# emmanuel-ferdman/pinot

Measured on AMD Instinct MI355X. Metric: rows scanned/s (G) + p50 query latency, SSB flattened SF100/SF1000, 1-8 GPU, higher is better.
Workload: dtype u32 dict ids / int64 sums; 1 GPU; SSB SF100 flattened lineorder per GPU, 100 segments x 6000000 rows, queries Q1.1+Q1.2+Q1.3; layout=sorted by LO_ORDERDATE (SURVEY.md §8d C2), rows_per_gpu=600000000, parallelism=one GPU (no collective)

## Files before the change

### pinot_amd/csrc/agg_kernel.h

```cpp
#pragma once
#include <hip/hip_ext.h>

#include "agg_common.h"

namespace phip {

struct HistCtx {
  lds_u32 *bins;
  int n;
};
template <int NA>
__device__ __forceinline__ void hist_flush(cquery_t &q, cseg_t &seg, uint64_t (&acc)[NA], HistCtx &hc) {
  const int lane = lane_id();
  ccol_t &c = seg.cols[q.hist_col];
#pragma unroll
  for (int a = 0; a < NA; a++) {
    if (a >= q.num_aggs) break;
    if (!((q.hist_aggs >> a) & 1u)) continue;
    const int kind = q.aggs[a].acc;
    if (kind == ACC_SUM_I64) {
      for (int i = lane; i < c.card; i += 64) {
        const uint32_t cnt = (hc.bins[i >> 1] >> ((i & 1) * 16)) & 0xffffu;
        if (cnt) acc[a] += (uint64_t)cnt * (uint64_t)dict_i64(c, (uint32_t)i);
      }
// ... 655 lines not shown
  }
  HistCtx hc{nullptr, 0};
  if constexpr (kHist) {
    hc.bins = (lds_u32 *)rest + (size_t)hll_words + (size_t)wave * q.hist_words;
    for (int i = lane; i < q.hist_words; i += 64) hc.bins[i] = 0;
  }
  if (MODE == GB_LDS) {
    const int G = (int)q.num_groups;
    for (int i = threadIdx.x; i < q.tbl_words; i += kBlock) {
      const int row = i / G;
      uint64_t init = 0;
      if (row > 0 && q.aggs[row - 1].acc == ACC_MIN_F64) init = ~0ull;
      tbl[i] = init;
    }
    for (int i = threadIdx.x; i < q.hll_words; i += kBlock) hll_packed[i] = 0;
  }
  __syncthreads();

  const int x = blockIdx.x & 7;
  const int j = blockIdx.x >> 3;
  const int gx = gridDim.x >> 3;
  const int xs = (int)((int64_t)q.total_work * x / 8);
  const int xe = (int)((int64_t)q.total_work * (x + 1) / 8);
  const int wx = gx * W;
  const int wid = j * W + wave;

  uint64_t acc[NA];
#pragma unroll
  for (int a = 0; a < NA; a++) acc[a] = (a < q.num_aggs) ? acc_init(q.aggs[a].acc) : 0;

  cseg_t *segs = (cseg_t *)q.segs;
  const glb_u32 *mask = (const glb_u32 *)q.mask;
  int head = 0, tail = 0;
  int si = 0;
  int dict_si = -1;
  int t = xs + wid;
  constexpr int kMaskAhead = 4;
  uint32_t mq[kMaskAhead];
#pragma unroll
  for (int k = 0; k < kMaskAhead; k++)
    mq[k] = (mask != nullptr && t + k * wx < xe) ? __builtin_nontemporal_load(mask + (size_t)(t + k * wx) * 64 + lane) : 0u;
  for (; t < xe; t += wx) {
    const uint32_t m_raw = mq[0];
#pragma unroll
    for (int k = 0; k + 1 < kMaskAhead; k++) mq[k] = mq[k + 1];
    {
      const int tn = t + kMaskAhead * wx;
      mq[kMaskAhead - 1] = (mask != nullptr && tn < xe) ? __builtin_nontemporal_load(mask + (size_t)tn * 64 + lane) : 0u;
    }
    if (segs[si].work_begin + segs[si].num_work <= t) {
      if constexpr (MODE == GB_NONE) {
        if (head > tail) agg_ring_batch<NA, kHist>(q, segs[si], ring, tail, head - tail, acc, hll_lds, 0, &hc);
        if constexpr (kHist) hist_flush<NA>(q, segs[si], acc, hc);
      } else if constexpr (kGbBatch) {
        if (head > tail) group_ring_batch<MODE, kBatch, kRingGB, kRec>(q, segs[si], ring, tail, head - tail, tbl, hll_packed);
      } else if (head > tail) {
        const bool act = lane < head - tail;
        const int32_t doc = act ? (int32_t)ring[(tail + lane) & (R - 1)] : 0;
        do_chunk<NA, MODE, kRec>(q, segs[si], doc, act, acc, hll_lds, tbl, hll_packed);
      }
      head = tail = 0;
      while (si + 1 < q.num_segs && segs[si + 1].work_begin <= t) si++;
    }
    cseg_t &seg = segs[si];
    const int32_t doc0 = (seg.tile0 + (t - seg.work_begin)) * kTileDocs;
    const int32_t nvalid = min(kTileDocs, seg.num_docs - doc0);
    const uint32_t valid = valid_word(nvalid, lane);
    const uint32_t m = mask != nullptr ? (m_raw & valid) : valid;
    bool dense = ballot(m != valid) == 0;
    if constexpr (MODE == GB_NONE && kDense) {
      if (!dense) dense = wave_sum_u32((uint32_t)__popc(m)) >= (uint32_t)q.dense_min;
    }
    bool batched = false;
    if constexpr (MODE == GB_NONE && kDense) batched = dense;
    if constexpr (MODE == GB_NONE && kDense) {
    if (batched) {
      if (q.num_stage > 0) {
        if (dict_si != si) {
          for (int k = 0; k < q.num_stage; k++) {
            if (q.stage_dict_off[k] < 0) continue;
            ccol_t &c = seg.cols[q.stage_col[k]];
            if (!c.has_dict) continue;
            const int32_t nw = c.card * ((c.type == PHIP_TYPE_LONG || c.type == PHIP_TYPE_DOUBLE) ? 2 : 1);
            lds_u32 *dst = (lds_u32 *)(stg + q.stage_dict_off[k]);
            for (int i = lane; i < nw; i += 64) dst[i] = ((const glb_u32 *)c.dict)[i];
          }
          dict_si = si;
        }
        const int32_t tile = doc0 / kTileDocs;
        for (int k = 0; k < q.num_stage; k++) {
          ccol_t &c = seg.cols[q.stage_col[k]];
          if (!c.has_dict) continue;
          const int32_t nb = 256 * c.bits;
          const uint8_t *src = (const uint8_t *)c.words + (size_t)tile * nb + lane * 16;
          const uint32_t dst = stg_lds + (uint32_t)q.stage_off[k];
// ... 141 lines not shown
```

### pinot_amd/csrc/dev_common.h

```cpp
#pragma once
#include <hip/hip_runtime.h>

#include "../../include/pinot_hip.h"
#include "acc_ops.h"
#include "device.h"

namespace phip {

#define PHIP_CAS __attribute__((address_space(4)))
#define PHIP_GLB __attribute__((address_space(1)))
#define PHIP_LDS __attribute__((address_space(3)))
typedef const PHIP_CAS DevSeg cseg_t;
typedef const PHIP_CAS DevNode cnode_t;
typedef const PHIP_CAS DevCol ccol_t;

__device__ __forceinline__ int lane_id() { return threadIdx.x & 63; }

__device__ __forceinline__ uint64_t ballot(bool p) { return __ballot(p); }

__device__ __forceinline__ uint32_t mbcnt64(uint64_t m) {
  return __builtin_amdgcn_mbcnt_hi((uint32_t)(m >> 32), __builtin_amdgcn_mbcnt_lo((uint32_t)m, 0u));
}

__device__ __forceinline__ int uniform(int v) { return __builtin_amdgcn_readfirstlane(v); }

typedef uint32_t u32x2_a4 __attribute__((ext_vector_type(2), aligned(4)));
__device__ __forceinline__ uint32_t decode_bits(const uint32_t *words_generic, uint64_t off, uint32_t bits) {
  const PHIP_GLB u32x2_a4 *p = (const PHIP_GLB u32x2_a4 *)((const PHIP_GLB uint32_t *)words_generic + (off >> 5));
  const u32x2_a4 v = __builtin_nontemporal_load(p);
  const uint64_t win = ((uint64_t)v.x << 32) | (uint64_t)v.y;
  return (uint32_t)((win << (off & 31)) >> (64 - bits));
}

__device__ __forceinline__ uint32_t window_at(const PHIP_LDS uint32_t *w, int32_t p) {
  const int32_t q = (p - 1) >> 5;
  const uint32_t s = (uint32_t)(32 * (q + 1) - p);
  return __builtin_amdgcn_alignbit(w[q], w[q + 1], s);
}

#ifndef PHIP_DMA_POLICY
#define PHIP_DMA_POLICY "nt"
#endif
__device__ __forceinline__ void dma16(const uint8_t *gsrc, uint32_t lds_dst) {
  unsigned keep;
  asm volatile(
      "s_mov_b32 %0, m0\n\t"
      "s_mov_b32 m0, %2\n\t"
// ... 112 lines not shown
```

### pinot_amd/csrc/device.h

```cpp
#pragma once
#include <stdint.h>

#if defined(__HIPCC__)
#define PHIP_HD __host__ __device__
#else
#define PHIP_HD
#endif

namespace phip {

constexpr int kMaxQueryColumns = 16;
constexpr int kMaxAggs = 8;
constexpr int kRecKeys = 4;
constexpr int kRecFields = kRecKeys + 2 * kMaxAggs;
enum { REC_BITS = 0, REC_U16 = 1, REC_U32 = 2 };
struct RecSrc {
  const void *p;
  int32_t kind, bits, off, pad;
};
struct RecSrcs {
  RecSrc f[kRecFields];
};
constexpr int kMaxPrograms = 8;
constexpr int kDenseMin = 640;
// ... 207 lines not shown
  const int32_t *kf;
  uint64_t *segm;
  uint32_t *hll;
  uint64_t *out;
  uint32_t *counter;
  int32_t nba, na, nbf, nseg, hll_words, pad;
};

struct DevFilter {
  const DevSeg *segs;
  const DevNode *nodes;
  int32_t num_segs;
  int32_t total_work;
  int32_t stage_stride;
  int32_t nbuf;
  int32_t xcd_walk;
  int32_t min_dma;
  int32_t probe;
  int32_t contig_inline;
  uint32_t stats_programs;
  int32_t mask_nt;
  uint32_t *mask_out;
  uint64_t *partials;
  uint64_t *seg_matched;
  const struct DevAggQuery *agg;
  uint64_t *agg_partials;
  int32_t fring_bytes;
  int32_t pad_f;
  const DevFinal *fin;
  uint64_t *rec;
  const int32_t *rec_first;
  int32_t rec_stride;
  uint32_t rec_tag;
};

struct DevAgg {
  int32_t acc;
  int32_t expr;
  int32_t col_a;
  int32_t col_b;
  int32_t integral;
  int32_t hll_slot;
  int32_t log2m;
  int32_t program;
};

struct DevAggQuery {
  const DevSeg *segs;
  int32_t num_segs;
  int32_t total_work;
  const uint32_t *mask;
  int32_t num_aggs;
  int32_t num_hll;
  int32_t log2m;
  int32_t mode;
  DevAgg aggs[kMaxAggs];
  int32_t num_group_by;
  int32_t gb_cols[kMaxGroupBy];
  int32_t dense_batch;
  int64_t gb_stride[kMaxGroupBy];
  int64_t num_groups;
  int32_t tbl_words;
  int32_t hll_words;
  uint64_t *gb_table;
  uint32_t *gb_hll;
  uint64_t *partials;
  uint32_t *hll_regs;
  int32_t stage_bytes;
  int32_t num_stage;
  int32_t stage_col[kMaxAggStage];
  int32_t stage_off[kMaxAggStage];
  int32_t stage_dict_off[kMaxAggStage];
  int32_t stage_slot_a[kMaxAggs];
  int32_t stage_slot_b[kMaxAggs];
  uint64_t *gb_keys;
  uint32_t *hash_overflow;
  int32_t seg_keys;
  int32_t seg_key_mult;
  uint32_t *first_doc;
  int32_t dense_min;
  int32_t own_count_rows;
  const DevFinal *fin;
  int32_t wg_waves;
  int32_t rec_on;
  int64_t xcd_words;
  int64_t xcd_hll_words;
  int8_t rec_fa[kMaxAggs];
  int8_t rec_fb[kMaxAggs];
  uint32_t hist_aggs;
  int32_t hist_col;
  int32_t hist_words;
  int32_t hist_pad;
};

constexpr int kMaxSelect = 16;
enum SelKind : int32_t {
  SEL_I64 = 0,
  SEL_F64 = 1,
  SEL_ID = 2,
  SEL_STR = 3,
};
struct DevSelect {
  int32_t expr;
  int32_t col_a;
  int32_t col_b;
  int32_t kind;
};
struct DevSelQuery {
  const DevSeg *segs;
  int32_t num_segs;
  int32_t total_work;
  const uint32_t *mask;
  const int64_t *tile_off;
  const int64_t *seg_base;
  int64_t limit;
  int32_t num_select;
  int32_t pad;
  DevSelect sel[kMaxSelect];
};

constexpr int kMaxDistinct = kMaxAggs;
constexpr int kDistinctLdsWords = 8192;
constexpr int kCountsCombineCard = 64;
constexpr int kCountsCombineRounds = 16;
struct DevDistinctQuery {
  const DevSeg *segs;
  int32_t num_segs;
  int32_t total_work;
  const uint32_t *mask;
  uint32_t *bitmap;
  int64_t num_rows;
  int64_t row_words;
  int32_t num_slots;
  int32_t lds;
  int32_t slot_col[kMaxDistinct];
  int32_t slot_card[kMaxDistinct];
  int32_t slot_kind[kMaxDistinct];
  int64_t slot_off[kMaxDistinct];
  int32_t num_group_by;
  int32_t combine_card;
  int32_t combine_rounds;
  int32_t gb_cols[kMaxGroupBy];
  int64_t gb_stride[kMaxGroupBy];
};

constexpr int kMaxOrderKeys = 8;
struct KeyOrder {
  int32_t num_group_by;
  int32_t num_keys;
  int32_t gb[kMaxOrderKeys];
  int32_t desc[kMaxOrderKeys];
  int64_t card[kMaxOrderKeys];
};

enum OrderTermKind : int32_t { TERM_GROUP_KEY = 0, TERM_VALUE = 1, TERM_AVG = 2, TERM_RANGE = 3, TERM_HLL = 4 };
struct OrderTerms {
  int32_t num_group_by;
  int32_t num_terms;
  int64_t card[kMaxOrderKeys];
  int32_t kind[kMaxOrderKeys];
  int32_t a[kMaxOrderKeys];
  int32_t b[kMaxOrderKeys];
  int32_t desc[kMaxOrderKeys];
};

struct RawChunk {
  uint64_t src;
  uint64_t dst;
  uint32_t csize;
  uint32_t usize;
};

struct RoaringTask {
  const uint8_t *payload;
  uint64_t *out_words;
  int32_t key;
// ... 15 lines not shown
```

### pinot_amd/csrc/distinct.hip

```cpp
#include "agg_common.h"
#include "launch.h"

namespace phip {

typedef const PHIP_CAS DevDistinctQuery cdst_t;

constexpr int kDstBlock = 256;
constexpr int kDstWaves = kDstBlock / kWave;

__device__ __forceinline__ int32_t slot_words(cdst_t &q, int s) {
  return q.slot_kind[s] == PHIP_DISTINCT_SLOT_COUNTS ? q.slot_card[s] : (q.slot_card[s] + 31) >> 5;
}

__device__ __forceinline__ int64_t distinct_key(cdst_t &q, cseg_t &seg, int32_t doc) {
  int64_t key = 0;
  for (int k = 0; k < q.num_group_by; k++) {
    ccol_t &c = seg.cols[q.gb_cols[k]];
    const uint32_t id = col_dict_id(c, doc);
    const int64_t gid = c.remap ? ((const PHIP_GLB int32_t *)c.remap)[id] : (int32_t)id;
    key += gid * q.gb_stride[k];
  }
  return key;
}

__device__ __forceinline__ void mark_global(uint32_t *word, uint32_t bit) {
  glb_u32 *p = (glb_u32 *)word;
  if (__hip_atomic_load(p, PHIP_RLX, PHIP_AG) & bit) return;
  (void)__hip_atomic_fetch_or(p, bit, PHIP_RLX, PHIP_AG);
}

template <bool kLds>
__global__ __launch_bounds__(kDstBlock) void distinct_mark_kernel(const DevDistinctQuery *qp) {
  extern __shared__ uint32_t dst_lds[];
  cdst_t &q = *(cdst_t *)qp;
  cseg_t *segs = (cseg_t *)q.segs;
  const int lane = lane_id();
  const int wave = uniform(threadIdx.x >> 6);
  const int32_t row_words = (int32_t)q.row_words;
  if (kLds) {
    for (int32_t i = threadIdx.x; i < row_words; i += kDstBlock) dst_lds[i] = 0u;
    __syncthreads();
  }
  const int64_t nw = (int64_t)gridDim.x * kDstWaves, w = (int64_t)blockIdx.x * kDstWaves + wave;
  const int b = (int)((int64_t)q.total_work * w / nw), e = (int)((int64_t)q.total_work * (w + 1) / nw);
  int si = 0;
  for (int t = b; t < e; t++) {
    while (si + 1 < q.num_segs && segs[si + 1].work_begin <= t) si++;
    cseg_t &seg = segs[si];
    const int32_t doc0 = (seg.tile0 + (t - seg.work_begin)) * kTileDocs;
    const uint32_t valid = valid_word(min(kTileDocs, seg.num_docs - doc0), lane);
    const uint32_t m =
        q.mask != nullptr ? (((const PHIP_GLB uint32_t *)q.mask)[(size_t)t * 64 + lane] & valid) : valid;
    uint32_t any = wave_or32(m);
    while (any) {
      const int g = __builtin_clz(any);
      any &= ~(0x80000000u >> g);
      if (!((m << g) & 0x80000000u)) continue;
      const int32_t doc = doc0 + 64 * g + lane;
      const int64_t key = q.num_group_by > 0 ? distinct_key(q, seg, doc) : 0;
      if (key < 0 || key >= q.num_rows) continue;
      for (int s = 0; s < q.num_slots; s++) {
        ccol_t &c = seg.cols[q.slot_col[s]];
        const uint32_t id = col_dict_id(c, doc);
        const uint32_t gid = c.remap ? (uint32_t)((const PHIP_GLB int32_t *)c.remap)[id] : id;
        if (gid >= (uint32_t)q.slot_card[s]) continue;
        if (q.slot_kind[s] == PHIP_DISTINCT_SLOT_COUNTS) {
          const uint64_t w = (kLds ? 0ull : (uint64_t)key * (uint64_t)q.row_words) + (uint64_t)q.slot_off[s] + gid;
          uint32_t add = 1u;
          if (!kLds && q.slot_card[s] <= q.combine_card) {
            bool pending = true;
            for (int r = 0; r < q.combine_rounds && pending; r++) {
              const uint32_t lo = (uint32_t)__builtin_amdgcn_readfirstlane((int)(uint32_t)w);
              const uint32_t hi = (uint32_t)__builtin_amdgcn_readfirstlane((int)(uint32_t)(w >> 32));
              const bool mine = w == (((uint64_t)hi << 32) | lo);
              const uint64_t same = ballot(mine);
              if (mine) {
                add = mbcnt64(same) == 0 ? (uint32_t)__popcll(same) : 0u;
                pending = false;
              }
            }
// ... 77 lines not shown
```

### pinot_amd/csrc/filter_kernel.h

```cpp
#pragma once
#include <hip/hip_ext.h>

#include "agg_kernel.h"
#include "host_final.h"

namespace phip {

struct Tile {
  int32_t doc0;
  int32_t valid_docs;
  const PHIP_LDS uint8_t *stage;
};

#define PHIP_GROUP_LOOP(PASS_EXPR)                                             \
  const int lane = lane_id();                                                  \
  const int32_t p = lane * B;                                                  \
  const int32_t q = (p - 1) >> 5;                                              \
  const uint32_t s = (uint32_t)(32 * (q + 1) - p);                             \
  const PHIP_LDS uint32_t *wl = w + q;                                         \
  const int32_t gstride = 2 * B;                                               \
  uint32_t r = 0;                                                              \
  _Pragma("unroll 8") for (int g = 0; g < kTileGroups; g++) {                  \
    const uint32_t win = __builtin_amdgcn_alignbit(wl[0], wl[1], s);           \
    wl += gstride;                                                             \
// ... 1110 lines not shown
  const int head0 = head;
  const int npiece = head - tail + r.total <= kFusedRingGB ? 1 : 16;
  const int lanes = 64 / npiece;
  for (int p = 0; p < npiece; p++) {
    const int e = __builtin_amdgcn_readlane((int)r.incl, lanes * p + lanes - 1);
    write_ranked<uint32_t, kFusedRingGB>(r, lanes * p, lanes * (p + 1), -head0, t.doc0, ring);
    head = head0 + e;
    while (head - tail >= kGbFlush) {
      fused_flush_gb<MODE>(aq, seg, ring, tail, kGbFlush, tbl, hll_packed);
      tail += kGbFlush;
    }
  }
}

#define PHIP_VMW(k) \
  case k: asm volatile("s_waitcnt vmcnt(" #k ")" ::: "memory"); break;
__device__ __forceinline__ void wait_vmcnt_lb(int n) {
  switch (__builtin_amdgcn_readfirstlane(n)) {
    PHIP_VMW(0) PHIP_VMW(1) PHIP_VMW(2) PHIP_VMW(3) PHIP_VMW(4) PHIP_VMW(5) PHIP_VMW(6) PHIP_VMW(7)
    PHIP_VMW(8) PHIP_VMW(9) PHIP_VMW(10) PHIP_VMW(11) PHIP_VMW(12) PHIP_VMW(13) PHIP_VMW(14)
    default: asm volatile("s_waitcnt vmcnt(15)" ::: "memory"); break;
  }
}
#undef PHIP_VMW

template <int kS>
struct StageCursor {
  const uint8_t *ptr[kS];
  int32_t bytes[kS];
  int32_t lds[kS];
  int32_t n;
};

template <int kS>
__device__ __forceinline__ void cursor_load(StageCursor<kS> &c, cseg_t &seg, int32_t tile_in_seg) {
  c.n = seg.num_stage;
#pragma unroll
  for (int i = 0; i < kS; i++) {
    c.ptr[i] = nullptr;
    c.bytes[i] = 0;
    c.lds[i] = 0;
    if (i < c.n) {
      c.bytes[i] = seg.stage[i].bytes;
      c.lds[i] = seg.stage[i].lds_off;
      c.ptr[i] = seg.stage[i].base + (int64_t)tile_in_seg * c.bytes[i];
    }
  }
}

template <int kS>
__device__ __forceinline__ void cursor_issue(StageCursor<kS> &c, uint32_t lbase, int step) {
  const int lane16 = lane_id() * 16;
#pragma unroll
  for (int i = 0; i < kS; i++) {
    if (i < c.n) {
      const uint8_t *g = c.ptr[i] + lane16;
      const uint32_t l = lbase + (uint32_t)c.lds[i];
      const int32_t nb = c.bytes[i];
      for (int off = 0; off < nb; off += 1024) {
        if (off + lane16 < nb) dma16(g + off, l + (uint32_t)off);
      }
      c.ptr[i] += (int64_t)nb * step;
    }
  }
}

template <int NA>
__device__ __forceinline__ void record_store(const DevFilter &q, const uint64_t *part, const uint64_t *apart,
                                             const uint32_t *segrow) {
  const int i = (int)threadIdx.x;
  if (i >= (q.rec_stride >> 3)) return;
  int na = 0;
  if constexpr (NA > 0) na = ((cquery_t *)q.agg)->num_aggs;
  uint64_t v = 0;
  if (i < 2) {
    for (int w = 0; w < kFilterWaves; w++) v += part[w * 2 + i];
  } else if (i < 2 + 2 * na) {
    if constexpr (NA > 0) {
// ... 52 lines not shown
  const int st = kBsDefer ? 0 : (q.mask_out != nullptr ? 1 : 0);
  constexpr int NAX = NA > 0 ? NA : 1;
  constexpr int kB = kBsDefer ? lean_batch(NA) : kFusedBatch;
  constexpr int kGbMode = NA == kFusedGroupByXcd ? GB_XCD : (NA == kFusedGroupByLds ? GB_LDS : GB_GLOBAL);
  lds_u64 *gtbl = nullptr;
  lds_u32 *ghll = nullptr;
  if constexpr (NA == kFusedGroupByLds) {
    cquery_t &aq = *(cquery_t *)q.agg;
    gtbl = (lds_u64 *)(smem + (size_t)kFilterWaves * (nbuf * stride + q.fring_bytes));
    ghll = (lds_u32 *)((PHIP_LDS uint8_t *)gtbl + (size_t)aq.tbl_words * 8);
    const int G = (int)aq.num_groups;
    for (int i = threadIdx.x; i < aq.tbl_words; i += kFilterBlock) {
      const int row = i / G;
      gtbl[i] = (row > 0 && aq.aggs[row - 1].acc == ACC_MIN_F64) ? ~0ull : 0ull;
    }
    for (int i = threadIdx.x; i < aq.hll_words; i += kFilterBlock) ghll[i] = 0;
    __syncthreads();
  }
  __shared__ uint32_t segrow[kFilterWaves][NA >= 0 ? kRecSegSlots : 1];
  if constexpr (NA >= 0) {
    segrow[wave][min(lane, kRecSegSlots - 1)] = 0;
  }
  uint64_t acc[NAX];
  SmallDict sda[NAX], sdb[NAX];
  if constexpr (NA > 0) {
    cquery_t &aq = *(cquery_t *)q.agg;
#pragma unroll
    for (int a = 0; a < NA; a++) {
      acc[a] = a < aq.num_aggs ? acc_init(aq.aggs[a].acc) : 0;
      sda[a] = sdb[a] = SmallDict{0u, 0u, false};
    }
  }

  int pf = begin, pfc = 0, psn = 0, pend = -1, pslot = 0;
  StageCursor<kS> cur;
  cur.n = 0;
#define PHIP_PREFETCH()                                                                         \
  do {                                                                                          \
    if (pf >= pend) {                                                                           \
      while (psn + 1 < q.num_segs && segs[psn].work_begin + segs[psn].num_work <= pf) psn++;    \
      cseg_t &ps = segs[psn];                                                                   \
      pend = ps.work_begin + ps.num_work;                                                       \
      cursor_load<kS>(cur, ps, ps.tile0 + (pf - ps.work_begin));                                \
    }                                                                                           \
    cursor_issue<kS>(cur, ring_lds + (uint32_t)(pslot * stride), step);                         \
    pf += step;                                                                                 \
    pfc++;                                                                                      \
    pslot = pslot + 1 == nbuf ? 0 : pslot + 1;                                                  \
  } while (0)
  for (int i = 0; i < nbuf - 1 && pf < end; i++) PHIP_PREFETCH();

  int si = -1;
  int seg_end = -1;
  int slot = 0;
  int k = 0;
  for (int t = begin; t < end; t += step, k++) {
    if (pf < end) PHIP_PREFETCH();
    if (t >= seg_end) {
      if constexpr (NA > 0) {
        if (si >= 0 && dhead > dtail)
          fused_flush<NA, kB>(*(cquery_t *)q.agg, segs[si], deferring, dtail, dhead - dtail, sda, sdb, acc);
        dhead = dtail = 0;
      }
      if constexpr (NA < 0) {
        while (si >= 0 && dhead > dtail) {
          fused_flush_gb<kGbMode>(*(cquery_t *)q.agg, segs[si], deferring, dtail, min(dhead - dtail, kGbFlush), gtbl,
                                  ghll);
          dtail += kGbFlush;
        }
        dhead = dtail = 0;
      }
      if (si >= 0) {
        const uint64_t m = wave_reduce_u64_add(lane_matched);
        lane_matched = 0;
        matched_total += m;
        if (NA >= 0 && q.seg_matched == nullptr) {
          if (lane == 0) segrow[wave][si % kRecSegSlots] = (uint32_t)m;
        } else if (m && lane == 0) {
          atomicAdd((unsigned long long *)&q.seg_matched[segs[si].seg_index], (unsigned long long)m);
        }
      }
      si = si < 0 ? 0 : si;
      while (si + 1 < q.num_segs && segs[si + 1].work_begin <= t) si++;
      seg_end = segs[si].work_begin + segs[si].num_work;
      if constexpr (NA > 0) {
        cquery_t &aq = *(cquery_t *)q.agg;
#pragma unroll
        for (int a = 0; a < NA; a++) {
          if (a >= aq.num_aggs || aq.aggs[a].acc == ACC_COUNT) continue;
          sda[a] = load_small_dict(segs[si].cols[aq.aggs[a].col_a]);
          if (aq.aggs[a].expr != PHIP_EXPR_COLUMN) sdb[a] = load_small_dict(segs[si].cols[aq.aggs[a].col_b]);
        }
      }
    }
    cseg_t &seg = segs[si];
    Tile tl;
    const int32_t tile_in_seg = seg.tile0 + (t - seg.work_begin);
    tl.doc0 = tile_in_seg * kTileDocs;
    tl.valid_docs = min(kTileDocs, seg.num_docs - tl.doc0);
    tl.stage = ring + slot * stride;
    wait_vmcnt_lb((pfc - k - 1) * nd + min(k, nbuf - 1) * st);

    const uint32_t valid = valid_word(tl.valid_docs, lane);
    uint32_t scanned_t = 0;
    uint32_t mask;
    if (q.probe) {
      mask = valid;
    } else if (kConjOnly || seg.conj_path) {
      if constexpr (kBsDefer) mask = seg.conj > 0 ? (valid & eval_conj_bs(seg, tl.stage)) : valid;
      else mask = seg.conj > 0 ? eval_conj(seg, tl.stage, valid) : valid;
      if (seg.conj_range && (seg.conj_lo > tl.doc0 || seg.conj_hi < tl.doc0 + kTileDocs - 1)) {
        const int32_t lo = max(seg.conj_lo - tl.doc0, 0), hi = min(seg.conj_hi - tl.doc0, kTileDocs - 1);
        mask &= lo <= hi ? range_word(lo, hi, lane) : 0u;
      }
      scanned_t = (uint32_t)seg.conj * (uint32_t)tl.valid_docs;
// ... 118 lines not shown
```

### pinot_amd/csrc/runtime.cpp

```cpp
#include <hip/hip_runtime.h>

#include <algorithm>
#include <atomic>
#include <chrono>
#include <condition_variable>
#include <cmath>
#include <cstdarg>
#include <cstdio>
#include <cstring>
#include <functional>
#include <map>
#include <memory>
#include <mutex>
#include <string>
#include <unordered_map>
#include <vector>

#include "../../include/pinot_hip.h"
#include "device.h"
#include "host_final.h"
#include "launch.h"
#include "node.h"

using namespace phip;
// ... 3346 lines not shown
    num_entries++;
    if (hull_lo > hull_hi) continue;
    ds.tile0 = (int32_t)(hull_lo / kTileDocs);
    ds.num_work = (int32_t)(hull_hi / kTileDocs - ds.tile0 + 1);
    ds.work_begin = (int32_t)total_work;
    total_work += ds.num_work;
    dsegs.push_back(ds);
   }
  }
  if (hll_made) HIP_TRY(hipStreamSynchronize(st));
  if (total_work > INT32_MAX / 2) return fail(PHIP_ERR_UNSUPPORTED, "too many tiles in one query");
  dq.total_work = (int32_t)total_work;
  if (group_by && gb_key_space > ((int64_t)1 << 22) && tl_node_docs == 0) {
    const int64_t work_docs = std::max<int64_t>(1, total_work * (int64_t)kTileDocs);
    if (gb_force_hash || gb_key_space > ((int64_t)1 << 26) || gb_key_space > 4 * work_docs) {
      const int64_t bound = std::max<int64_t>(1, std::min<int64_t>(gb_key_space, work_docs));
      int64_t cap = 1024;
      while (cap < 2 * bound) cap <<= 1;
      if (const char *hc = getenv("PHIP_GB_HASH_CAP"))
        cap = std::max<int64_t>(64, std::min<int64_t>(cap, (int64_t)1 << (63 - __builtin_clzll((uint64_t)std::max(2LL, atoll(hc))))));
      if (dq.mode != GB_HASH || cap < dq.num_groups) {
        const int64_t per_slot = 8 + 8 * (1 + (int64_t)naggs);
        if (cap * per_slot > ((int64_t)24 << 30))
          return fail(PHIP_ERR_UNSUPPORTED, "group-by hash table of %lld slots exceeds the memory budget", (long long)cap);
        dq.num_groups = cap;
        dq.mode = GB_HASH;
      }
    }
  }
  if (!P.dist_agg.empty() && group_by && dq.mode == GB_HASH)
    return fail(PHIP_ERR_UNSUPPORTED, "DISTINCTCOUNT / value counts over a hash-table group-by key space");
  dq.num_segs = (int32_t)dsegs.size();
  const size_t segs_off = blob.reserve(sizeof(DevSeg) * std::max<size_t>(dsegs.size(), 1));

  std::vector<RoaringTask> tasks;
  size_t inv_words_total = 0;
  std::vector<size_t> inv_word_off(inv_leaves.size()), inv_word_nw(inv_leaves.size());
  std::vector<int> entry_leaves(num_entries, 0);
  std::vector<size_t> entry_off(num_entries, 0);
  for (const InvLeaf &L : inv_leaves) entry_leaves[L.entry]++;
  for (size_t i = 0; i < inv_leaves.size(); i++) {
    const InvLeaf &L = inv_leaves[i];
    const Segment &sg = *segs[L.seg];
    size_t nw = (size_t)std::max(round_up(sg.num_docs, 65536), round_up(sg.num_docs, kTileDocs)) / 64;
    inv_word_nw[i] = nw;
    if (L.slot == 0) {
      entry_off[L.entry] = inv_words_total;
      inv_words_total += nw * entry_leaves[L.entry];
    }
    inv_word_off[i] = entry_off[L.entry] + 32 * (size_t)L.slot;
  }
  std::vector<int32_t> node_inv_stride(nodes.size(), 0);
  std::vector<int32_t> node_inv_slot(nodes.size(), 0);
  std::vector<int32_t> node_inv_leaves(nodes.size(), 0);
  void *inv_words = nullptr;
  if (inv_words_total) {
    int32_t rc = P.alloc(inv_words_total * 8, &inv_words);
    if (rc) return rc;
  }
  std::vector<RoaringGroup> rgroups;
  for (size_t i = 0; i < inv_leaves.size(); i++) {
    const InvLeaf &L = inv_leaves[i];
    const ColumnStore &cs = segs[L.seg]->cols[L.col];
    uint64_t *words = (uint64_t *)inv_words + inv_word_off[i];
    const int32_t tile_words = 32 * entry_leaves[L.entry];
    nodes[L.node].aux = words;
// ... 517 lines not shown
      dq.rec_on = any_rec ? 1 : 0;
      P.walk_adaptive = (nhll == 0 || any_rec) && !gbb && !gw && !fused_gb && P.walk[0].ok && P.walk[1].ok;
      P.walk_cur = batched ? 1 : 0;
    }
  } else if (nhll) {
    agg_lds += (size_t)nhll * m_regs * 4;
  }
  if (!group_by && dq.hist_aggs) agg_lds += (size_t)kAggWaves * dq.hist_words * 4;
  if (dq.wg_waves == 0) dq.wg_waves = kAggWaves;
  if (dq.mode != GB_LDS || fused_gb) {
    dq.rec_on = 0;
    for (DevSeg &d : dsegs) d.rec = nullptr;
  }
  int agg_blocks = (int)std::min<int64_t>((int64_t)grid_cus * agg_bpc, ceil_div(total_work, dq.wg_waves));
  agg_blocks = (int)round_up(std::max(agg_blocks, 8), 8);
  if (P.walk_cur >= 0) agg_blocks = P.walk[P.walk_cur].blocks;

  const size_t nodes_off = blob.reserve(std::max<size_t>(nodes.size(), 1) * sizeof(DevNode));
  kinds[naggs] = ACC_COUNT;
  kinds[naggs + 1] = ACC_COUNT;
  const size_t kinds_off = blob.add(kinds.data(), kinds.size() * 4);
  const size_t dq_off = blob.reserve(sizeof(DevAggQuery));
  const size_t sq_off = nsel > 0 ? blob.reserve(sizeof(DevSelQuery)) : 0;
  const size_t dstq_off = ndist > 0 ? blob.reserve(sizeof(DevDistinctQuery)) : 0;

  void *dblob;
  int32_t rc = P.alloc(blob.data.size() + 64, &dblob);
  if (rc) return rc;
  uint8_t *base = (uint8_t *)dblob;
  for (auto &f : aux_fix) nodes[f.node].aux = base + f.off;
  if (!nodes.empty()) memcpy(blob.data.data() + nodes_off, nodes.data(), nodes.size() * sizeof(DevNode));
  if (!dsegs.empty()) memcpy(blob.data.data() + segs_off, dsegs.data(), sizeof(DevSeg) * dsegs.size());
  const DevSeg *dev_segs = (const DevSeg *)(base + segs_off);

  DevFilter fq;
  memset(&fq, 0, sizeof(fq));
  fq.segs = dev_segs;
  fq.nodes = (const DevNode *)(base + nodes_off);
  fq.num_segs = (int32_t)dsegs.size();
  fq.total_work = (int32_t)total_work;
  fq.stage_stride = stage_stride;
  fq.nbuf = nbuf;
  fq.fring_bytes = fring_bytes;
  fq.xcd_walk = xcd_walk;
  {
    const char *pe = getenv("PHIP_FILTER_PROBE");
    fq.probe = pe ? atoi(pe) : 0;
    const char *ie = getenv("PHIP_CONTIG_INLINE");
    fq.contig_inline = ie ? atoi(ie) : 1;
  }
  fq.stats_programs = q->stats_programs ? (uint32_t)q->stats_programs : 0xffffffffu;
  {
    const char *mn = getenv("PHIP_MASK_NT");
    fq.mask_nt = mn ? atoi(mn) : 0;
  }
  fq.min_dma = 0;
  for (size_t i = 0; i < dsegs.size(); i++)
    fq.min_dma = i == 0 ? dsegs[i].num_dma : std::min(fq.min_dma, dsegs[i].num_dma);
  dq.segs = dev_segs;

  void *fpart, *finals, *seg_matched, *apart = nullptr, *masks = nullptr;
  rc = P.alloc((size_t)filter_blocks * 2 * 8, &fpart);
  if (rc) return rc;
  const int nmatch = nprog * nseg;
  rc = P.alloc((64 + (size_t)nmatch) * 8 + (size_t)std::max(nhll, 1) * (1 << 12) * 4, &finals);
  if (rc) return rc;
  seg_matched = (uint64_t *)finals + 64;
  fq.partials = (uint64_t *)fpart;
  fq.seg_matched = (uint64_t *)seg_matched;
  dq.hll_regs = (uint32_t *)((uint64_t *)finals + 64 + nmatch);
  if (need_mask) {
    rc = P.alloc((size_t)std::max<int64_t>(total_work, 1) * 64 * 4, &masks);
    if (rc) return rc;
    fq.mask_out = (uint32_t *)masks;
    dq.mask = (const uint32_t *)masks;
  }
  if (need_agg && !group_by) {
    const int pblocks = fused_naggs > 0 ? filter_blocks : agg_blocks;
    rc = P.alloc((size_t)pblocks * std::max(naggs, 1) * 8, &apart);
    if (rc) return rc;
    dq.partials = (uint64_t *)apart;
    if (fused_naggs > 0) {
      fq.agg_partials = (uint64_t *)apart;
      fq.agg = (const DevAggQuery *)(base + dq_off);
    }
  }
  if (fused_gb) fq.agg = (const DevAggQuery *)(base + dq_off);
  void *gtab = nullptr, *ghll = nullptr, *slab = nullptr, *hslab = nullptr;
  if (group_by) {
    const size_t copies = gb_xcd ? kXcdCopies : 1;
    rc = P.alloc(copies * (1 + naggs) * dq.num_groups * 8, &gtab);
    if (rc) return rc;
// ... 12 lines not shown
      rc = P.alloc(16, &ho);
      if (rc) return rc;
      dq.gb_keys = (uint64_t *)hk;
      dq.hash_overflow = (uint32_t *)ho;
    }
    if (dq.mode == GB_LDS) {
      const size_t nslabs = gb_lds ? filter_blocks
                                   : std::max<int>(agg_blocks, P.walk_adaptive ? std::max(P.walk[0].blocks, P.walk[1].blocks) : 0);
      rc = P.alloc(nslabs * dq.tbl_words * 8 + 16, &slab);
      if (rc) return rc;
      if (nhll) {
        rc = P.alloc(nslabs * dq.hll_words * 4 + 16, &hslab);
        if (rc) return rc;
      }
      dq.gb_table = (uint64_t *)slab;
      dq.gb_hll = (uint32_t *)hslab;
    } else {
      dq.gb_table = (uint64_t *)gtab;
      dq.gb_hll = (uint32_t *)ghll;
    }
  }
  void *fo = nullptr;
  if (want_bitmap) {
    rc = P.alloc((size_t)filter_nwords * 8 + 4096 * 8, &fo);
    if (rc) return rc;
  }

  memcpy(blob.data.data() + dq_off, &dq, sizeof(dq));
  if (ndist > 0) {
    P.dist_bytes = (size_t)dstq.num_rows * (size_t)dstq.row_words * 4;
    rc = P.alloc(P.dist_bytes, &P.dist_bits);
    if (rc) return rc;
    dstq.segs = dev_segs;
    dstq.num_segs = (int32_t)dsegs.size();
    dstq.total_work = (int32_t)total_work;
    dstq.mask = need_mask ? (const uint32_t *)masks : nullptr;
    dstq.bitmap = (uint32_t *)P.dist_bits;
    memcpy(blob.data.data() + dstq_off, &dstq, sizeof(dstq));
    P.ndist = ndist;
    P.dstq = dstq;
    P.dstq_off = dstq_off;
    P.dist_lds_bytes = dstq.lds ? (size_t)round_up(std::max<int64_t>(dstq.row_words, 1) * 4, 16) : 0;
    P.dist_blocks = grid_cus * (dstq.lds ? 4 : 8);
    for (auto &e : P.dist_ev) HIP_TRY(hipEventCreate(&e));
  }
  if (nsel > 0) {
    void *sb;
    const size_t nent = dsegs.size();
    rc = P.alloc(((size_t)total_work + 1) * 16 + (2 * nent + 1) * 8 + 16, &sb);
    if (rc) return rc;
    P.sel_tile_cnt = (int64_t *)sb;
    P.sel_tile_off = P.sel_tile_cnt + total_work + 1;
    P.sel_base = P.sel_tile_off + total_work + 1;
    P.sel_kept = P.sel_base + nent + 1;
    P.sel_total = P.sel_kept + nent;
    sq.segs = dev_segs;
    sq.num_segs = (int32_t)nent;
    sq.total_work = (int32_t)total_work;
    sq.mask = has_filter ? (const uint32_t *)masks : nullptr;
    sq.tile_off = P.sel_tile_off;
    sq.seg_base = P.sel_base;
    memcpy(blob.data.data() + sq_off, &sq, sizeof(sq));
    P.select = true;
    P.nsel = nsel;
    P.sq_off = sq_off;
    P.sel_types = sel_types;
    P.sel_dicts = sel_dicts;
    P.sel_str_ptrs.assign(nsel, {});
    for (int k = 0; k < nsel; k++) {
      if (sq.sel[k].kind != SEL_STR) continue;
      std::vector<const void *> &v = P.sel_str_ptrs[k];
      v.resize(2 * (size_t)nseg);
      for (int s = 0; s < nseg; s++) {
        const ColumnStore &cs = segs[s]->cols[colidx[s][sq.sel[k].col_a]];
        v[s] = cs.raw;
        v[nseg + s] = cs.str_off;
      }
    }
    for (int k = 0; k < nsel; k++) {
      for (int c : {sq.sel[k].col_a, sq.sel[k].expr != PHIP_EXPR_COLUMN ? sq.sel[k].col_b : -1}) {
        if (c < 0) continue;
        const ColumnStore &cs = segs[0]->cols[colidx[0][c]];
        P.sel_bits.push_back(no_dict(cs) ? 0 : cs.bits);
        P.sel_width.push_back(cs.type == PHIP_TYPE_STRING ? 4 : type_width(cs.type));
      }
    }
  }
  HIP_TRY(hipMemcpyAsync(dblob, blob.data.data(), blob.data.size(), hipMemcpyHostToDevice, st));
  HIP_TRY(hipStreamSynchronize(st));
// ... 2096 lines not shown
```

### pinot_amd/csrc/select.hip

```cpp
#include <hipcub/hipcub.hpp>

#include "agg_common.h"
#include "launch.h"

namespace phip {

typedef const PHIP_CAS DevSelQuery csel_t;

constexpr int kSelBlock = 256;
constexpr int kSelWaves = kSelBlock / kWave;

__device__ __forceinline__ uint32_t sel_tile_mask(csel_t &q, cseg_t &seg, int t) {
  const int32_t doc0 = (seg.tile0 + (t - seg.work_begin)) * kTileDocs;
  const uint32_t valid = valid_word(min(kTileDocs, seg.num_docs - doc0), lane_id());
  return q.mask != nullptr ? (((const PHIP_GLB uint32_t *)q.mask)[(size_t)t * 64 + lane_id()] & valid) : valid;
}

__global__ __launch_bounds__(kSelBlock) void select_count_kernel(const DevSelQuery *qp, int64_t *__restrict__ tile_cnt) {
  csel_t &q = *(csel_t *)qp;
  cseg_t *segs = (cseg_t *)q.segs;
  const int64_t nw = (int64_t)gridDim.x * kSelWaves, w = (int64_t)blockIdx.x * kSelWaves + (threadIdx.x >> 6);
  const int b = (int)((int64_t)q.total_work * w / nw), e = (int)((int64_t)q.total_work * (w + 1) / nw);
  int si = 0;
  for (int t = b; t < e; t++) {
    while (si + 1 < q.num_segs && segs[si + 1].work_begin <= t) si++;
    const uint32_t n = wave_sum_u32((uint32_t)__popc(sel_tile_mask(q, segs[si], t)));
    if (lane_id() == 0) tile_cnt[t] = n;
  }
  if (blockIdx.x == 0 && threadIdx.x == 0) tile_cnt[q.total_work] = 0;
}

__global__ void select_bases_kernel(const DevSelQuery *qp, int64_t *__restrict__ seg_base, int64_t *__restrict__ kept,
                                    int64_t *__restrict__ total) {
  csel_t &q = *(csel_t *)qp;
  if (threadIdx.x != 0) return;
  cseg_t *segs = (cseg_t *)q.segs;
  int64_t run = 0;
  for (int e = 0; e < q.num_segs; e++) {
    const int64_t m = q.tile_off[segs[e].work_begin + segs[e].num_work] - q.tile_off[segs[e].work_begin];
    const int64_t k = m < q.limit ? m : q.limit;
    seg_base[e] = run;
    kept[e] = k;
    run += k;
  }
  seg_base[q.num_segs] = run;
  total[0] = run < q.limit ? run : q.limit;
  total[1] = run;
}

__device__ __forceinline__ uint64_t sel_value(cseg_t &seg, const PHIP_CAS DevSelect &s, int32_t doc) {
  ccol_t &a = seg.cols[s.col_a];
  if (s.expr == PHIP_EXPR_COLUMN) {
    if (s.kind == SEL_ID) {
      const uint32_t id = col_dict_id(a, doc);
      return (uint64_t)(int64_t)(a.remap ? ((const PHIP_GLB int32_t *)a.remap)[id] : (int32_t)id);
    }
    if (s.kind == SEL_STR) return ((uint64_t)(uint32_t)seg.seg_index << 32) | (uint32_t)doc;
    if (s.kind == SEL_I64) return (uint64_t)col_i64(a, doc);
    return as_u64(col_f64(a, doc));
  }
  const double x = col_f64(a, doc), y = col_f64(seg.cols[s.col_b], doc);
  return as_u64(s.expr == PHIP_EXPR_ADD ? x + y : (s.expr == PHIP_EXPR_SUB ? x - y : x * y));
}

__global__ __launch_bounds__(kSelBlock) void select_gather_kernel(const DevSelQuery *qp, uint64_t *__restrict__ out,
                                                                  int64_t num_rows) {
  __shared__ uint16_t ring_all[kSelWaves][kTileDocs];
  csel_t &q = *(csel_t *)qp;
  cseg_t *segs = (cseg_t *)q.segs;
  const int lane = lane_id();
  const int wave = uniform(threadIdx.x >> 6);
  uint16_t *ring = ring_all[wave];
  const int64_t nw = (int64_t)gridDim.x * kSelWaves, w = (int64_t)blockIdx.x * kSelWaves + wave;
  const int b = (int)((int64_t)q.total_work * w / nw), e = (int)((int64_t)q.total_work * (w + 1) / nw);
  int si = 0;
  for (int t = b; t < e; t++) {
    while (si + 1 < q.num_segs && segs[si + 1].work_begin <= t) si++;
    cseg_t &seg = segs[si];
    const int64_t rank0 = q.tile_off[t] - q.tile_off[seg.work_begin];
    const int64_t row0 = q.seg_base[si] + rank0;
    if (rank0 >= q.limit || row0 >= num_rows) continue;
    const uint32_t m = sel_tile_mask(q, seg, t);
    if (ballot(m != 0) == 0) continue;
    uint32_t cw = lane_major_to_contig(m);
    const uint32_t cnt = (uint32_t)__popc(cw);
    const uint32_t incl = wave_incl_scan(cnt);
    const int total = __builtin_amdgcn_readlane((int)incl, 63);
    int pos = (int)(incl - cnt);
    while (cw) {
      const int j = __builtin_clz(cw);
      cw &= ~(0x80000000u >> j);
      ring[pos++] = (uint16_t)(32 * lane + j);
    }
    __builtin_amdgcn_wave_barrier();
    const int32_t doc0 = (seg.tile0 + (t - seg.work_begin)) * kTileDocs;
    for (int c = 0; c < total; c += 64) {
      const int i = c + lane;
      const int64_t rank = rank0 + i, row = row0 + i;
      const bool act = i < total && rank < q.limit && row < num_rows;
      const int32_t doc = doc0 + (act ? (int32_t)ring[i] : 0);
      for (int k = 0; k < q.num_select; k++) {
        const uint64_t v = sel_value(seg, q.sel[k], doc);
        if (act) out[(size_t)k * (size_t)num_rows + (size_t)row] = v;
      }
    }
    __builtin_amdgcn_wave_barrier();
  }
}

static inline int sel_blocks(int64_t total_work, int max_blocks) {
// ... 60 lines not shown
```

Baseline: 10840 G rows/s.

## Seed segment index via binary search over compact seg_begin array

Adds a compact int32 array of per-segment work begins, built and validated on the host. Kernels use it to binary-search each wave's starting segment instead of linearly walking the DevSeg structs from zero, and advance through it with cheaper scalar loads. The filter kernel also gains a wide vector load of the stage descriptors for the cursor. The aim is to cut the per-wave segment-walk cost and scattered scalar loads of large DevSeg records. The host now rejects work lists with non-contiguous segments.

```diff
diff --git a/pinot_amd/csrc/agg_kernel.h b/pinot_amd/csrc/agg_kernel.h
--- a/pinot_amd/csrc/agg_kernel.h
+++ b/pinot_amd/csrc/agg_kernel.h
@@ -711,9 +711,10 @@
   cseg_t *segs = (cseg_t *)q.segs;
   const glb_u32 *mask = (const glb_u32 *)q.mask;
   int head = 0, tail = 0;
-  int si = 0;
   int dict_si = -1;
   int t = xs + wid;
+  csegbeg_t sbeg = (csegbeg_t)q.seg_begin;
+  int si = t < xe ? seg_of_tile(sbeg, q.num_segs, t) : 0;
   constexpr int kMaskAhead = 4;
   uint32_t mq[kMaskAhead];
 #pragma unroll
@@ -727,7 +728,7 @@
       const int tn = t + kMaskAhead * wx;
       mq[kMaskAhead - 1] = (mask != nullptr && tn < xe) ? __builtin_nontemporal_load(mask + (size_t)tn * 64 + lane) : 0u;
     }
-    if (segs[si].work_begin + segs[si].num_work <= t) {
+    if (sbeg[si + 1] <= t) {
       if constexpr (MODE == GB_NONE) {
         if (head > tail) agg_ring_batch<NA, kHist>(q, segs[si], ring, tail, head - tail, acc, hll_lds, 0, &hc);
         if constexpr (kHist) hist_flush<NA>(q, segs[si], acc, hc);
@@ -739,7 +740,7 @@
         do_chunk<NA, MODE, kRec>(q, segs[si], doc, act, acc, hll_lds, tbl, hll_packed);
       }
       head = tail = 0;
-      while (si + 1 < q.num_segs && segs[si + 1].work_begin <= t) si++;
+      si = seg_of_tile(sbeg, q.num_segs, t);
     }
     cseg_t &seg = segs[si];
     const int32_t doc0 = (seg.tile0 + (t - seg.work_begin)) * kTileDocs;
diff --git a/pinot_amd/csrc/dev_common.h b/pinot_amd/csrc/dev_common.h
--- a/pinot_amd/csrc/dev_common.h
+++ b/pinot_amd/csrc/dev_common.h
@@ -4,6 +4,7 @@
 #include "../../include/pinot_hip.h"
 #include "acc_ops.h"
 #include "device.h"
+#include "seg_lookup.h"
 
 namespace phip {
 
@@ -13,6 +14,7 @@
 typedef const PHIP_CAS DevSeg cseg_t;
 typedef const PHIP_CAS DevNode cnode_t;
 typedef const PHIP_CAS DevCol ccol_t;
+typedef const PHIP_CAS int32_t *csegbeg_t;
 
 __device__ __forceinline__ int lane_id() { return threadIdx.x & 63; }
 
diff --git a/pinot_amd/csrc/device.h b/pinot_amd/csrc/device.h
--- a/pinot_amd/csrc/device.h
+++ b/pinot_amd/csrc/device.h
@@ -263,6 +263,7 @@
   const int32_t *rec_first;
   int32_t rec_stride;
   uint32_t rec_tag;
+  const int32_t *seg_begin;
 };
 
 struct DevAgg {
@@ -322,6 +323,7 @@
   int32_t hist_col;
   int32_t hist_words;
   int32_t hist_pad;
+  const int32_t *seg_begin;
 };
 
 constexpr int kMaxSelect = 16;
@@ -348,6 +350,7 @@
   int32_t num_select;
   int32_t pad;
   DevSelect sel[kMaxSelect];
+  const int32_t *seg_begin;
 };
 
 constexpr int kMaxDistinct = kMaxAggs;
@@ -373,6 +376,7 @@
   int32_t combine_rounds;
   int32_t gb_cols[kMaxGroupBy];
   int64_t gb_stride[kMaxGroupBy];
+  const int32_t *seg_begin;
 };
 
 constexpr int kMaxOrderKeys = 8;
diff --git a/pinot_amd/csrc/distinct.hip b/pinot_amd/csrc/distinct.hip
--- a/pinot_amd/csrc/distinct.hip
+++ b/pinot_amd/csrc/distinct.hip
@@ -43,9 +43,10 @@
   }
   const int64_t nw = (int64_t)gridDim.x * kDstWaves, w = (int64_t)blockIdx.x * kDstWaves + wave;
   const int b = (int)((int64_t)q.total_work * w / nw), e = (int)((int64_t)q.total_work * (w + 1) / nw);
-  int si = 0;
+  csegbeg_t sbeg = (csegbeg_t)q.seg_begin;
+  int si = b < e ? seg_of_tile(sbeg, q.num_segs, b) : 0;
   for (int t = b; t < e; t++) {
-    while (si + 1 < q.num_segs && segs[si + 1].work_begin <= t) si++;
+    si = seg_advance(sbeg, si, t);
     cseg_t &seg = segs[si];
     const int32_t doc0 = (seg.tile0 + (t - seg.work_begin)) * kTileDocs;
     const uint32_t valid = valid_word(min(kTileDocs, seg.num_docs - doc0), lane);
diff --git a/pinot_amd/csrc/filter_kernel.h b/pinot_amd/csrc/filter_kernel.h
--- a/pinot_amd/csrc/filter_kernel.h
+++ b/pinot_amd/csrc/filter_kernel.h
@@ -1166,18 +1166,29 @@
   int32_t n;
 };
 
-template <int kS>
+typedef uint32_t stage_words_t __attribute__((ext_vector_type(4), aligned(8)));
+template <int kS, bool kWide>
 __device__ __forceinline__ void cursor_load(StageCursor<kS> &c, cseg_t &seg, int32_t tile_in_seg) {
+  static_assert(kS <= kMaxStage && sizeof(StageSrc) == sizeof(stage_words_t), "DevSeg.stage: kMaxStage 16-byte sources");
   c.n = seg.num_stage;
-#pragma unroll
-  for (int i = 0; i < kS; i++) {
-    c.ptr[i] = nullptr;
-    c.bytes[i] = 0;
-    c.lds[i] = 0;
-    if (i < c.n) {
-      c.bytes[i] = seg.stage[i].bytes;
-      c.lds[i] = seg.stage[i].lds_off;
-      c.ptr[i] = seg.stage[i].base + (int64_t)tile_in_seg * c.bytes[i];
+  if constexpr (kWide) {
+    const PHIP_CAS stage_words_t *sw = (const PHIP_CAS stage_words_t *)seg.stage;
+    stage_words_t w[kS];
+#pragma unroll
+    for (int i = 0; i < kS; i++) w[i] = sw[i];
+#pragma unroll
+    for (int i = 0; i < kS; i++) {
+      c.bytes[i] = (int32_t)w[i][2];
+      c.lds[i] = (int32_t)w[i][3];
+      c.ptr[i] = (const uint8_t *)(uintptr_t)(((uint64_t)w[i][1] << 32) | w[i][0]) + (int64_t)tile_in_seg * c.bytes[i];
+    }
+  } else {
+#pragma unroll
+    for (int i = 0; i < kS; i++) {
+      const bool on = i < c.n;
+      c.bytes[i] = on ? seg.stage[i].bytes : 0;
+      c.lds[i] = on ? seg.stage[i].lds_off : 0;
+      c.ptr[i] = on ? seg.stage[i].base + (int64_t)tile_in_seg * seg.stage[i].bytes : nullptr;
     }
   }
 }
@@ -1296,16 +1307,19 @@
     }
   }
 
-  int pf = begin, pfc = 0, psn = 0, pend = -1, pslot = 0;
+  csegbeg_t sbeg = (csegbeg_t)q.seg_begin;
+  const int seed = begin < end ? seg_of_tile(sbeg, q.num_segs, begin) : 0;
+  int pf = begin, pfc = 0, psn = seed, pend = -1, pslot = 0;
   StageCursor<kS> cur;
   cur.n = 0;
+  constexpr bool kWideCursor = kBsDefer || NA >= 2;
 #define PHIP_PREFETCH()                                                                         \
   do {                                                                                          \
     if (pf >= pend) {                                                                           \
       while (psn + 1 < q.num_segs && segs[psn].work_begin + segs[psn].num_work <= pf) psn++;    \
       cseg_t &ps = segs[psn];                                                                   \
       pend = ps.work_begin + ps.num_work;                                                       \
-      cursor_load<kS>(cur, ps, ps.tile0 + (pf - ps.work_begin));                                \
+      cursor_load<kS, kWideCursor>(cur, ps, ps.tile0 + (pf - ps.work_begin));                   \
     }                                                                                           \
     cursor_issue<kS>(cur, ring_lds + (uint32_t)(pslot * stride), step);                         \
     pf += step;                                                                                 \
@@ -1314,7 +1328,7 @@
   } while (0)
   for (int i = 0; i < nbuf - 1 && pf < end; i++) PHIP_PREFETCH();
 
-  int si = -1;
+  int si = ~seed;
   int seg_end = -1;
   int slot = 0;
   int k = 0;
@@ -1344,7 +1358,7 @@
           atomicAdd((unsigned long long *)&q.seg_matched[segs[si].seg_index], (unsigned long long)m);
         }
       }
-      si = si < 0 ? 0 : si;
+      si = si < 0 ? ~si : si;
       while (si + 1 < q.num_segs && segs[si + 1].work_begin <= t) si++;
       seg_end = segs[si].work_begin + segs[si].num_work;
       if constexpr (NA > 0) {
diff --git a/pinot_amd/csrc/runtime.cpp b/pinot_amd/csrc/runtime.cpp
--- a/pinot_amd/csrc/runtime.cpp
+++ b/pinot_amd/csrc/runtime.cpp
@@ -3402,6 +3402,16 @@
     return fail(PHIP_ERR_UNSUPPORTED, "DISTINCTCOUNT / value counts over a hash-table group-by key space");
   dq.num_segs = (int32_t)dsegs.size();
   const size_t segs_off = blob.reserve(sizeof(DevSeg) * std::max<size_t>(dsegs.size(), 1));
+  std::vector<int32_t> seg_begin(dsegs.size() + 1);
+  for (size_t i = 0; i < dsegs.size(); i++) {
+    const int64_t next = i + 1 < dsegs.size() ? dsegs[i + 1].work_begin : total_work;
+    if (dsegs[i].num_work < 1 || dsegs[i].work_begin + (int64_t)dsegs[i].num_work != next)
+      return fail(PHIP_ERR_INVALID, "work-list entry %d: tiles [%d, +%d) do not meet the next entry's", (int)i,
+                  dsegs[i].work_begin, dsegs[i].num_work);
+    seg_begin[i] = dsegs[i].work_begin;
+  }
+  seg_begin[dsegs.size()] = (int32_t)total_work;
+  const size_t seg_begin_off = blob.add(seg_begin.data(), seg_begin.size() * 4, 64);
 
   std::vector<RoaringTask> tasks;
   size_t inv_words_total = 0;
@@ -3985,10 +3995,12 @@
   if (!nodes.empty()) memcpy(blob.data.data() + nodes_off, nodes.data(), nodes.size() * sizeof(DevNode));
   if (!dsegs.empty()) memcpy(blob.data.data() + segs_off, dsegs.data(), sizeof(DevSeg) * dsegs.size());
   const DevSeg *dev_segs = (const DevSeg *)(base + segs_off);
+  const int32_t *dev_seg_begin = (const int32_t *)(base + seg_begin_off);
 
   DevFilter fq;
   memset(&fq, 0, sizeof(fq));
   fq.segs = dev_segs;
+  fq.seg_begin = dev_seg_begin;
   fq.nodes = (const DevNode *)(base + nodes_off);
   fq.num_segs = (int32_t)dsegs.size();
   fq.total_work = (int32_t)total_work;
@@ -4011,6 +4023,7 @@
   for (size_t i = 0; i < dsegs.size(); i++)
     fq.min_dma = i == 0 ? dsegs[i].num_dma : std::min(fq.min_dma, dsegs[i].num_dma);
   dq.segs = dev_segs;
+  dq.seg_begin = dev_seg_begin;
 
   void *fpart, *finals, *seg_matched, *apart = nullptr, *masks = nullptr;
   rc = P.alloc((size_t)filter_blocks * 2 * 8, &fpart);
@@ -4089,6 +4102,7 @@
     rc = P.alloc(P.dist_bytes, &P.dist_bits);
     if (rc) return rc;
     dstq.segs = dev_segs;
+    dstq.seg_begin = dev_seg_begin;
     dstq.num_segs = (int32_t)dsegs.size();
     dstq.total_work = (int32_t)total_work;
     dstq.mask = need_mask ? (const uint32_t *)masks : nullptr;
@@ -4112,6 +4126,7 @@
     P.sel_kept = P.sel_base + nent + 1;
     P.sel_total = P.sel_kept + nent;
     sq.segs = dev_segs;
+    sq.seg_begin = dev_seg_begin;
     sq.num_segs = (int32_t)nent;
     sq.total_work = (int32_t)total_work;
     sq.mask = has_filter ? (const uint32_t *)masks : nullptr;
diff --git a/pinot_amd/csrc/seg_lookup.h b/pinot_amd/csrc/seg_lookup.h
--- /dev/null
+++ b/pinot_amd/csrc/seg_lookup.h
@@ -0,0 +1,25 @@
+#pragma once
+#include <stdint.h>
+
+#include "device.h"
+
+namespace phip {
+
+template <typename Ptr>
+PHIP_HD inline int seg_of_tile(Ptr seg_begin, int n, int t) {
+  int lo = 0;
+  for (int len = n; len > 1;) {
+    const int half = len >> 1;
+    lo = seg_begin[lo + half] <= t ? lo + half : lo;
+    len -= half;
+  }
+  return lo;
+}
+
+template <typename Ptr>
+PHIP_HD inline int seg_advance(Ptr seg_begin, int si, int t) {
+  while (seg_begin[si + 1] <= t) si++;
+  return si;
+}
+
+}
diff --git a/pinot_amd/csrc/select.hip b/pinot_amd/csrc/select.hip
--- a/pinot_amd/csrc/select.hip
+++ b/pinot_amd/csrc/select.hip
@@ -21,9 +21,10 @@
   cseg_t *segs = (cseg_t *)q.segs;
   const int64_t nw = (int64_t)gridDim.x * kSelWaves, w = (int64_t)blockIdx.x * kSelWaves + (threadIdx.x >> 6);
   const int b = (int)((int64_t)q.total_work * w / nw), e = (int)((int64_t)q.total_work * (w + 1) / nw);
-  int si = 0;
+  csegbeg_t sbeg = (csegbeg_t)q.seg_begin;
+  int si = b < e ? seg_of_tile(sbeg, q.num_segs, b) : 0;
   for (int t = b; t < e; t++) {
-    while (si + 1 < q.num_segs && segs[si + 1].work_begin <= t) si++;
+    si = seg_advance(sbeg, si, t);
     const uint32_t n = wave_sum_u32((uint32_t)__popc(sel_tile_mask(q, segs[si], t)));
     if (lane_id() == 0) tile_cnt[t] = n;
   }
@@ -73,9 +74,10 @@
   uint16_t *ring = ring_all[wave];
   const int64_t nw = (int64_t)gridDim.x * kSelWaves, w = (int64_t)blockIdx.x * kSelWaves + wave;
   const int b = (int)((int64_t)q.total_work * w / nw), e = (int)((int64_t)q.total_work * (w + 1) / nw);
-  int si = 0;
+  csegbeg_t sbeg = (csegbeg_t)q.seg_begin;
+  int si = b < e ? seg_of_tile(sbeg, q.num_segs, b) : 0;
   for (int t = b; t < e; t++) {
-    while (si + 1 < q.num_segs && segs[si + 1].work_begin <= t) si++;
+    si = seg_advance(sbeg, si, t);
     cseg_t &seg = segs[si];
     const int64_t rank0 = q.tile_off[t] - q.tile_off[seg.work_begin];
     const int64_t row0 = q.seg_base[si] + rank0;
```

Measured after the change: 10860 G rows/s, median of 3. Within noise of the previous version (+0.1%).
